# dwkim606/optimal_conv

Hardware: AMD Instinct MI355X
Metric: homomorphic convs/sec (conv_then_pack + BN bias, k x k, batch B, N=2^16) (higher is better)
Workload: dtype u64; 1 GPU; conv 3 3; ker_wid=3, batch=256, in_wid=16, logN=16, moduli=ckks.DefaultBootstrapParams[6] Q0,Q1 + P=0x1fffffffffe00001, ciphertexts_per_launch_set=4, contexts_per_gpu=4, chunk_nodes=512

## Files before the change

### optimal_conv_amd/csrc/hc_kernels.h

```cpp
#pragma once
#include "hc_arith.h"

#define HC_TPB 256
#ifndef HC_MIN_WAVES
#define HC_MIN_WAVES 4
#endif
#define HC_ROWS_LDS 4096
#define HC_COLS_LDS 4096

struct __attribute__((aligned(16))) HcTw { u64 w, ws; };

#define HC_SMALL_Q(q) ((q) < (1ull << 31))
template <bool B> struct HcBool { static constexpr bool value = B; };
template <int V> struct HcInt { static constexpr int value = V; };
#define HC_COUNT_DISPATCH(n, body) do { switch (n) { case 1: body(HcInt<1>{}); break; case 2: body(HcInt<2>{}); break; case 3: body(HcInt<3>{}); break; case 4: body(HcInt<4>{}); break; \
    case 5: body(HcInt<5>{}); break; case 6: body(HcInt<6>{}); break; case 7: body(HcInt<7>{}); break; case 8: body(HcInt<8>{}); break; default: break; } } while (0)
#define HC_LD(S32, rowptr, j) ((S32) ? hc_ld32(rowptr, j) : (rowptr)[j])
#define HC_ST(S32, rowptr, j, v) do { if (S32) hc_st32(rowptr, j, v); else (rowptr)[j] = (v); } while (0)
#define HC_ROW_DISPATCH(row32, body) do { if (row32) body(HcBool<true>{}); else body(HcBool<false>{}); } while (0)
__device__ __forceinline__ u64 hc_ld32(const u64 *row, size_t j) { return (u64)reinterpret_cast<const u32 *>(row)[j]; }
__device__ __forceinline__ void hc_st32(u64 *row, size_t j, u64 v) { reinterpret_cast<u32 *>(row)[j] = (u32)v; }
struct __attribute__((packed, aligned(4))) HcU64A4 { u64 v; };
__device__ __forceinline__ u64 hc_ldp(const u64 *row, size_t j, bool row32) {
    return reinterpret_cast<const HcU64A4 *>(reinterpret_cast<const char *>(row) + (j << (row32 ? 2 : 3)))->v & (row32 ? 0xFFFFFFFFull : ~0ull);
// ... 795 lines not shown
    const HcTw *__restrict__ c0 = A.ctc + ((size_t)z * 4 + 1) * 65536 + (size_t)HC_TILE * 4096 + t;
    const u64 *__restrict__ k = A.ker.p[z] + ((size_t)i * 2 + 1) * 65536 + (size_t)HC_TILE * 4096 + t;
    const HcQ Q = hc_q(A.m1.q);
    const HcTw wA = hc_twl_load(T1inv, HC_TILE, t);
    u64 e0[16], e1[16];
#pragma unroll
    for (int kk = 0; kk < 16; kk++) {
        const u64 kv = k[kk * 256];
        const HcTw w0 = c0[kk * 256], w1 = c0[2 * 65536 + kk * 256];
        e0[kk] = hc_shoup4(kv, w0.w, w0.ws, Q);
        e1[kk] = hc_shoup4(kv, w1.w, w1.ws, Q);
    }
    u64 *o = A.tmp + ((size_t)z * A.njobs + 2 * ch) * 65536 + (size_t)row * 256;
    hc_xchg(lds, [&](int kk) { return hc_rows_lds(kk, t); }, [&](int lo) { return hc_rows_lds(rloc, tid * 16 + lo); }, [] { __syncthreads(); }, e0, e1);
    HC_ROW_SYNC();
    if (F64) {
        const HcF64Mod m{(double)A.m1.q, 1.0 / (double)A.m1.q};
        double f0[16], f1[16];
#pragma unroll
        for (int kk = 0; kk < 16; kk++) { f0[kk] = hc_f64_reduce(hc_f64_from_u(e0[kk]), m.q, m.qinv); f1[kk] = hc_f64_reduce(hc_f64_from_u(e1[kk]), m.q, m.qinv); }
        hc_rows_inv2_f64(f0, f1, lds, T1inv, wA, row, rloc, tid, m);
#pragma unroll
        for (int hi = 0; hi < 16; hi++) { o[hi * 16 + tid] = hc_d2u(f0[hi]); o[65536 + hi * 16 + tid] = hc_d2u(f1[hi]); }
    } else {
        hc_rows_inv_twl(HcLazy<>{Q}, lds, T1inv, wA, row, rloc, tid, e0, e1);
#pragma unroll
        for (int hi = 0; hi < 16; hi++) { o[hi * 16 + tid] = e0[hi]; o[65536 + hi * 16 + tid] = e1[hi]; }
    }
}
template <int FM, int F64>
__global__ __launch_bounds__(HC_TPB, HC_W_A2) void hc_k_a2(HcLoopA A, HcTwTab T1inv, HcTwTab T0fwd) {
    __shared__ u32 lds[HC_COLS_LDS];
    __shared__ __attribute__((aligned(16))) HcTw twl[HC_COLS_TWL];
    const int t = threadIdx.x, c = t & 15, tid = t >> 4;
    u64 *base = A.tmp + (size_t)HC_JOB * 65536 + HC_TILE * 16 + c;
    const HcQ Q0 = hc_q(A.m0.q);
    const HcTw wI = hc_twc_load(T1inv, t), wF = hc_twc_load(T0fwd, t);
    u64 e[16];
#pragma unroll
    for (int lo = 0; lo < 16; lo++) e[lo] = base[(size_t)(tid * 16 + lo) * 256];
    const HcTwC tI = hc_twc_put(twl, 0, wI, t), tF = hc_twc_put(twl, 1, wF, t);
    HC_ROW_SYNC();
    if (F64) {
        const double q1 = (double)A.m1.q, hh = (double)A.h;
        const HcF64Mod m{q1, 1.0 / q1};
        double f[16];
#pragma unroll
        for (int lo = 0; lo < 16; lo++) f[lo] = hc_u2d(e[lo]);
        hc_cols_inv_f64(f, lds, T1inv, tI, c, tid, m);
#pragma unroll
        for (int hi = 0; hi < 16; hi++) {
            double v = f[hi];
            v = v > hh ? v - q1 : (v < -hh ? v + q1 : v);
            e[hi] = hc_f64_to_u_plus(v, A.m0.q);
        }
    } else {
        const HcQ Q1 = hc_q(A.m1.q);
        hc_cols_inv_twl(HcLazy<>{Q1}, lds, T1inv, tI, c, tid, e, T1inv.ninv, T1inv.w_last_ninv);
#pragma unroll
        for (int hi = 0; hi < 16; hi++) {
            const u64 v = hc_csub(hc_canon4(e[hi], Q1) + A.h, A.m1.q);
            e[hi] = hc_reduce64(v + A.negh0, A.m0.mu, Q0);
        }
    }
    __syncthreads();
    hc_cols_fwd_twl(HcLazy<FM>{Q0}, lds, T0fwd, tF, c, tid, e);
#pragma unroll
    for (int lo = 0; lo < 16; lo++) base[(size_t)(tid * 16 + lo) * 256] = e[lo];
}
template <int FM>
__global__ __launch_bounds__(HC_TPB, HC_W_A3) void hc_k_a3p(HcLoopA A, HcTwTab T0fwd) {
    __shared__ __attribute__((aligned(16))) u64 lds[HC_ROWS_LDS];
    const int t = threadIdx.x, tid = t & 15, rloc = t >> 4, row = HC_TILE * 16 + rloc;
    const int ch = HC_JOB, i = A.i0 + ch * A.norm, z = blockIdx.z;
    const u64 *__restrict__ in = A.tmp + ((size_t)z * A.njobs + 2 * ch) * 65536 + (size_t)row * 256;
    const HcTw *__restrict__ c0 = A.ctc + (size_t)z * 4 * 65536 + (size_t)HC_TILE * 4096 + t;
    const u64 *__restrict__ k = A.ker.p[z] + ((size_t)i * 2) * 65536 + (size_t)HC_TILE * 4096 + t;
    u64 *__restrict__ o = A.cts + (size_t)z * A.cts_stride + (size_t)(A.slot0 + ch * A.slot_step) * 2 * 65536 + (size_t)HC_TILE * 4096 + t;
    const HcQ Q = hc_q(A.m0.q);
    const HcTw wA = hc_twl_load(T0fwd, HC_TILE, t);
    u64 e0[16], e1[16], kv[16];
#pragma unroll
    for (int hi = 0; hi < 16; hi++) { e0[hi] = in[hi * 16 + tid]; e1[hi] = in[65536 + hi * 16 + tid]; }
#pragma unroll
    for (int kk = 0; kk < 16; kk++) kv[kk] = k[kk * 256];
    hc_rows_fwd_twl(HcLazy<FM>{Q}, lds, T0fwd, wA, row, rloc, tid, e0, e1);
    HC_ROW_SYNC();
    hc_xchg(lds, [&](int lo) { return hc_rows_lds(rloc, tid * 16 + lo); }, [&](int kk) { return hc_rows_lds(kk, t); }, [] { __syncthreads(); }, e0, e1);
#pragma unroll
    for (int b = 0; b < 16; b += HC_A3_ROWS) {
        HcTw w0[HC_A3_ROWS], w1[HC_A3_ROWS];
#pragma unroll
        for (int j = 0; j < HC_A3_ROWS; j++) { w0[j] = c0[(b + j) * 256]; w1[j] = c0[2 * 65536 + (b + j) * 256]; }
#pragma unroll
        for (int j = 0; j < HC_A3_ROWS; j++) {
            const int kk = b + j;
            const u64 a0 = hc_shoup4(kv[kk], w0[j].w, w0[j].ws, Q), a1 = hc_shoup4(kv[kk], w1[j].w, w1[j].ws, Q);
            const u64 d0 = FM == HC_FM_FREE ? a0 + HC_FREE_OFF * Q.q - e0[kk] : a0 + Q.q - hc_canon8(e0[kk], Q);
            const u64 d1 = FM == HC_FM_FREE ? a1 + HC_FREE_OFF * Q.q - e1[kk] : a1 + Q.q - hc_canon8(e1[kk], Q);
            o[kk * 256] = hc_canon4(hc_shoup4(d0, A.q1inv.w, A.q1inv.ws, Q), Q);
            o[65536 + kk * 256] = hc_canon4(hc_shoup4(d1, A.q1inv.w, A.q1inv.ws, Q), Q);
        }
    }
}

struct HcLoopB {
    const u64 *src;
    u64 *dst;
    u64 *tmpC;
    u64 *tmpE;
    u64 *tmpT;
    const HcTw *idx;
    const HcTw *evkQ;
    const HcTw *evkP;
    const u64 *idxM;
    const u64 *evkQM;
    int n0, step, norm;
    int nodes;
    size_t src_stride, dst_stride;
    HcMod m0, mp;
    HcTw pmodq;
    HcTw pinv;
    u64 mu0;
    u64 vthresh;
    u32 gal;
};
__global__ __launch_bounds__(HC_TPB, HC_W_B1) void hc_k_b1(HcLoopB B, HcTwTab T0inv) {
    __shared__ __attribute__((aligned(16))) u64 lds[HC_ROWS_LDS];
    const int t = threadIdx.x, tid = t & 15, rloc = t >> 4, row = HC_TILE * 16 + rloc;
    const int job = HC_JOB, z = job / B.nodes, node = job - z * B.nodes, i = (B.n0 + node) * B.norm;
    const size_t tile = (size_t)HC_TILE * 4096 + t;
    const u64 *__restrict__ y1 = B.src + (size_t)z * B.src_stride + ((size_t)i * 2 + 1) * 65536 + tile;
    const u64 *__restrict__ x1 = B.src + (size_t)z * B.src_stride + ((size_t)(i + B.step) * 2 + 1) * 65536 + tile;
    const HcTw *__restrict__ idx = B.idx + tile;
    const HcQ Q = hc_q(B.m0.q);
    u64 e[16], yy[16];
#pragma unroll
    for (int kk = 0; kk < 16; kk++) { e[kk] = x1[kk * 256]; yy[kk] = y1[kk * 256]; }
#pragma unroll
    for (int kk = 0; kk < 16; kk++) {
        const HcTw I = idx[kk * 256];
        e[kk] = hc_fold(yy[kk] + Q.q4 - hc_shoup4(e[kk], I.w, I.ws, Q), Q.nq4);
    }
    if (B.tmpT != nullptr) {
        u64 *__restrict__ tt = B.tmpT + (size_t)job * 65536 + tile;
#pragma unroll
        for (int kk = 0; kk < 16; kk++) tt[kk * 256] = e[kk];
    }
    hc_rows_lin_to_lo(lds, t, rloc, tid, e);
    const HcTw wA = hc_twl_load(T0inv, HC_TILE, t);
    HC_ROW_SYNC();
    hc_rows_inv(HcLazy<>{Q}, lds, T0inv, row, rloc, tid, e, &wA);
    u64 *__restrict__ o = B.tmpC + (size_t)job * 65536 + (size_t)row * 256;
#pragma unroll
    for (int hi = 0; hi < 16; hi++) o[hi * 16 + tid] = e[hi];
}
template <int FMP>
__global__ __launch_bounds__(HC_TPB, HC_W_B2) void hc_k_b2(HcLoopB B, HcTwTab T0inv, HcTwTab TPfwd) {
    __shared__ u32 lds[HC_COLS_LDS];
    __shared__ __attribute__((aligned(16))) HcTw twl[HC_COLS_TWL];
    const int t = threadIdx.x, c = t & 15, tid = t >> 4;
    u64 *base = B.tmpC + (size_t)HC_JOB * 65536 + HC_TILE * 16 + c;
    const HcQ Q0 = hc_q(B.m0.q), QP = hc_q(B.mp.q);
    const HcTw wI = hc_twc_load(T0inv, t), wF = hc_twc_load(TPfwd, t);
    u64 e[16];
#pragma unroll
    for (int lo = 0; lo < 16; lo++) e[lo] = base[(size_t)(tid * 16 + lo) * 256];
    const HcTwC tI = hc_twc_put(twl, 0, wI, t), tF = hc_twc_put(twl, 1, wF, t);
    HC_ROW_SYNC();
    hc_cols_inv_twl(HcLazy<>{Q0}, lds, T0inv, tI, c, tid, e, T0inv.ninv, T0inv.w_last_ninv);
#pragma unroll
    for (int hi = 0; hi < 16; hi++) e[hi] = hc_canon4(e[hi], Q0);
    __syncthreads();
    hc_cols_fwd_twl(HcLazy<FMP>{QP}, lds, TPfwd, tF, c, tid, e);
#pragma unroll
    for (int lo = 0; lo < 16; lo++) base[(size_t)(tid * 16 + lo) * 256] = e[lo];
}
template <int FMP>
__global__ __launch_bounds__(HC_TPB, HC_W_B3) void hc_k_b3p(HcLoopB B, HcTwTab TPfwd, HcTwTab TPinv) {
    __shared__ __attribute__((aligned(16))) u64 lds[HC_ROWS_LDS];
    const int t = threadIdx.x, tid = t & 15, rloc = t >> 4, row = HC_TILE * 16 + rloc;
    const int node = HC_JOB;
    const u64 *in = B.tmpC + (size_t)node * 65536 + (size_t)row * 256;
    const HcQ Q = hc_q(B.mp.q);
    u64 e0[16], e1[16];
    HcTw wI;
    {
        const HcTw wA = hc_twl_load(TPfwd, HC_TILE, t);
        u64 cp[16];
#pragma unroll
        for (int hi = 0; hi < 16; hi++) cp[hi] = in[hi * 16 + tid];
        hc_rows_fwd_twl(HcLazy<FMP>{Q}, lds, TPfwd, wA, row, rloc, tid, cp);
        wI = hc_twl_load(TPinv, HC_TILE, t);
        const HcTw *__restrict__ ev = B.evkP + (size_t)HC_TILE * 4096 + t;
#pragma unroll
        for (int lo = 0; lo < 16; lo++) {
            const HcTw w0 = ev[lo * 256], w1 = ev[65536 + lo * 256];
            e0[lo] = hc_shoup4(cp[lo], w0.w, w0.ws, Q);
            e1[lo] = hc_shoup4(cp[lo], w1.w, w1.ws, Q);
        }
    }
    HC_ROW_SYNC();
    hc_rows_inv_twl(HcLazy<>{Q}, lds, TPinv, wI, row, rloc, tid, e0, e1);
    u64 *o = B.tmpE + (size_t)node * 2 * 65536 + (size_t)row * 256;
#pragma unroll
    for (int hi = 0; hi < 16; hi++) { o[hi * 16 + tid] = e0[hi]; o[65536 + hi * 16 + tid] = e1[hi]; }
}
template <int FM>
__global__ __launch_bounds__(HC_TPB, HC_W_B4) void hc_k_b4(HcLoopB B, HcTwTab TPinv, HcTwTab T0fwd) {
    __shared__ u32 lds[HC_COLS_LDS];
    __shared__ __attribute__((aligned(16))) HcTw twl[HC_COLS_TWL];
    const int t = threadIdx.x, c = t & 15, tid = t >> 4;
    u64 *base = B.tmpE + (size_t)HC_JOB * 65536 + HC_TILE * 16 + c;
    const HcQ QP = hc_q(B.mp.q), Q = hc_q(B.m0.q);
    const HcTw wI = hc_twc_load(TPinv, t), wF = hc_twc_load(T0fwd, t);
    u64 e[16];
#pragma unroll
    for (int lo = 0; lo < 16; lo++) e[lo] = base[(size_t)(tid * 16 + lo) * 256];
    const HcTwC tI = hc_twc_put(twl, 0, wI, t), tF = hc_twc_put(twl, 1, wF, t);
    HC_ROW_SYNC();
    hc_cols_inv_twl<false>(HcLazy<>{QP}, lds, TPinv, tI, c, tid, e, TPinv.ninv, TPinv.w_last_ninv);
#pragma unroll
    for (int hi = 0; hi < 16; hi++) {
        const u64 yv = hc_canon4(e[hi], QP);
        u64 r = hc_shoup4(yv, B.pinv.w, B.pinv.ws, Q);
        if (yv >= B.vthresh) r += Q.q - 1;
        e[hi] = r;
    }
    __syncthreads();
    hc_cols_fwd_twl(HcLazy<FM>{Q}, lds, T0fwd, tF, c, tid, e);
#pragma unroll
    for (int lo = 0; lo < 16; lo++) base[(size_t)(tid * 16 + lo) * 256] = e[lo];
}
template <int FM, int K0>
__device__ __forceinline__ void hc_b5_terms(u64 Y, u64 T, HcTw K, u64 X, HcTw I, const HcQ &Q, u64 &t1, u64 &f) {
    const u64 q = Q.q;
    u64 g = hc_shoup4(T, K.w, K.ws, Q);
    if (FM != HC_FM_FREE) g = hc_canon4(g, Q);
    if (K0) {
        u64 m = hc_shoup4(X, I.w, I.ws, Q);
        if (FM == HC_FM_FREE) { t1 = Y + m; f = Y + Q.q4 - m + g; }
        else { m = hc_canon4(m, Q); t1 = hc_addmod(Y, m, q); f = hc_addmod(hc_submod(Y, m, q), g, q); }
    } else {
        if (FM == HC_FM_FREE) t1 = Y + Y + Q.q4 - T;
        else t1 = hc_addmod(Y, hc_submod(Y, hc_canon4(T, Q), q), q);
        f = g;
    }
}
template <int FM>
__global__ __launch_bounds__(HC_TPB, 3) void hc_k_b5(HcLoopB B, HcTwTab T0fwd, HcPtrs biases, HcPtrs outs) {
    __shared__ u64 lds[HC_ROWS_LDS];
    const int t = threadIdx.x, tid = t & 15, rloc = t >> 4, row = HC_TILE * 16 + rloc;
    const int job = HC_JOB, zn = job >> 1, k = job & 1, z = zn / B.nodes, node = zn - z * B.nodes, i = (B.n0 + node) * B.norm;
    const HcQ Q = hc_q(B.m0.q);
    const u64 q = Q.q;
    const size_t tile = (size_t)HC_TILE * 4096 + t;
    const u64 *__restrict__ in = B.tmpE + (size_t)job * 65536 + (size_t)row * 256;
    const u64 *__restrict__ yk = B.src + (size_t)z * B.src_stride + ((size_t)i * 2 + k) * 65536 + tile;
    const u64 *__restrict__ xk = B.src + (size_t)z * B.src_stride + ((size_t)(i + B.step) * 2 + k) * 65536 + tile;
    const u64 *__restrict__ tc1 = B.tmpT + (size_t)zn * 65536 + tile;
    const HcTw *__restrict__ idx = B.idx + tile;
    const HcTw *__restrict__ evk = B.evkQ + (size_t)k * 65536 + tile;
    u64 *__restrict__ o = (outs.p[z] != nullptr ? const_cast<u64 *>(outs.p[z]) + (size_t)k * 65536 : B.dst + (size_t)z * B.dst_stride + ((size_t)i * 2 + k) * 65536) + tile;
    const u64 *__restrict__ bias = (k == 0 && biases.p[z] != nullptr) ? biases.p[z] + tile : nullptr;
    u64 e[16];
#pragma unroll
    for (int hi = 0; hi < 16; hi++) e[hi] = in[hi * 16 + tid];
    hc_rows_fwd(HcLazy<FM>{Q}, lds, T0fwd, row, rloc, tid, e);
    HC_ROW_SYNC();
    hc_rows_lo_to_lin(lds, t, rloc, tid, e);
    __syncthreads();
    {
        u64 t1[16];
#pragma unroll
        for (int b = 0; b < 16; b += 4) {
            u64 Y[4], T[4], X[4]; HcTw K[4], I[4];
#pragma unroll
            for (int j = 0; j < 4; j++) {
                const int off = (b + j) * 256;
                Y[j] = yk[off]; K[j] = evk[off]; T[j] = tc1[off];
                if (k == 0) { X[j] = xk[off]; I[j] = idx[off]; } else { X[j] = 0; I[j] = K[j]; }
            }
#pragma unroll
            for (int j = 0; j < 4; j++) {
                const int kk = b + j;
                u64 f;
                if (k == 0) hc_b5_terms<FM, 1>(Y[j], T[j], K[j], X[j], I[j], Q, t1[kk], f);
                else hc_b5_terms<FM, 0>(Y[j], T[j], K[j], X[j], I[j], Q, t1[kk], f);
                if (bias != nullptr) t1[kk] = FM == HC_FM_FREE ? t1[kk] + bias[kk * 256] : hc_addmod(t1[kk], bias[kk * 256], q);
                lds[hc_rows_lds(kk, t)] = FM == HC_FM_FREE ? f + HC_FREE_OFF * q - e[kk] : hc_submod(f, hc_canon8(e[kk], Q), q);
            }
        }
        __syncthreads();
#pragma unroll
        for (int kk = 0; kk < 16; kk++) {
            const u32 srcidx = hc_perm_src((u32)((HC_TILE * 16 + kk) * 256 + t), B.gal);
            const u64 d = lds[hc_rows_lds((int)((srcidx >> 8) & 15), (int)(srcidx & 255))];
            o[kk * 256] = FM == HC_FM_FREE ? hc_reduce64(t1[kk] + d, B.m0.mu, Q) : hc_addmod(t1[kk], d, q);
        }
    }
}

#ifndef HC_B5_ROWS
#define HC_B5_ROWS 4
#endif
#ifndef HC_B5M_WAVES
#define HC_B5M_WAVES 2
#endif
template <int FM>
__device__ __forceinline__ void hc_rows_fwd2_lin(u64 (&e0)[16], u64 (&e1)[16], u64 *l0, u64 *l1, const HcTwTab &T, const HcTw &wA, int row, int rloc, int tid, int t, const HcQ &Q) {
    hc_ct_round(HcLazy<FM>{Q}, hc_twl_put(l0, wA, rloc, tid), e0, e1);
    HC_ROW_SYNC();
#pragma unroll
    for (int hi = 0; hi < 16; hi++) { const int a = hc_rows_lds(rloc, hi * 16 + tid); l0[a] = e0[hi]; l1[a] = e1[hi]; }
    HC_ROW_SYNC();
#pragma unroll
    for (int lo = 0; lo < 16; lo++) { const int a = hc_rows_lds(rloc, tid * 16 + lo); e0[lo] = l0[a]; e1[lo] = l1[a]; }
    hc_ct_round(HcLazy<FM>{Q}, HcTwB<false, HcTw>{T.rowsB + row * 256 + tid}, e0, e1);
    HC_ROW_SYNC();
#pragma unroll
    for (int lo = 0; lo < 16; lo++) { const int a = hc_rows_lds(rloc, tid * 16 + lo); l0[a] = e0[lo]; l1[a] = e1[lo]; }
    __syncthreads();
#pragma unroll
    for (int k = 0; k < 16; k++) { const int a = hc_rows_lds(k, t); e0[k] = l0[a]; e1[k] = l1[a]; }
}
template <int FM>
__global__ __launch_bounds__(HC_TPB, HC_B5M_WAVES) void hc_k_b5m(HcLoopB B, HcTwTab T0fwd, HcPtrs biases, HcPtrs outs) {
    __shared__ __attribute__((aligned(16))) u64 lds[2 * HC_ROWS_LDS];
    u64 *l0 = lds, *l1 = lds + HC_ROWS_LDS;
    const int t = threadIdx.x, tid = t & 15, rloc = t >> 4, row = HC_TILE * 16 + rloc;
    const int zn = HC_JOB, z = zn / B.nodes, node = zn - z * B.nodes, i = (B.n0 + node) * B.norm;
    const HcQ Q = hc_q(B.m0.q);
    const u64 q = Q.q, qinv = B.m0.qinv;
    const size_t tile = (size_t)HC_TILE * 4096 + t;
    const u64 *__restrict__ ys = B.src + (size_t)z * B.src_stride + (size_t)i * 2 * 65536 + tile;
    const u64 *__restrict__ xs = B.src + (size_t)z * B.src_stride + (size_t)(i + B.step) * 2 * 65536 + tile;
    const u64 *__restrict__ idx = B.idxM + tile;
    const u64 *__restrict__ evk = B.evkQM + tile;
    u64 *__restrict__ o = (outs.p[z] != nullptr ? const_cast<u64 *>(outs.p[z]) : B.dst + (size_t)z * B.dst_stride + (size_t)i * 2 * 65536) + tile;
    const u64 *__restrict__ bias = biases.p[z] != nullptr ? biases.p[z] + tile : nullptr;
    const HcTw wA = hc_twl_load(T0fwd, HC_TILE, t);
    u64 e0[16], e1[16];
    {
        const u64 *__restrict__ in = B.tmpE + (size_t)zn * 2 * 65536 + (size_t)row * 256;
#pragma unroll
        for (int hi = 0; hi < 16; hi++) { e0[hi] = in[hi * 16 + tid]; e1[hi] = in[65536 + hi * 16 + tid]; }
    }
    hc_rows_fwd2_lin<FM>(e0, e1, l0, l1, T0fwd, wA, row, rloc, tid, t, Q);
    __syncthreads();
#pragma unroll
    for (int b = 0; b < 16; b += HC_B5_ROWS) {
        u64 Y0[HC_B5_ROWS], X0[HC_B5_ROWS], Y1[HC_B5_ROWS], X1[HC_B5_ROWS], K0[HC_B5_ROWS], K1[HC_B5_ROWS], I[HC_B5_ROWS], bs[HC_B5_ROWS], s0[HC_B5_ROWS], s1[HC_B5_ROWS];
#pragma unroll
        for (int j = 0; j < HC_B5_ROWS; j++) {
            const int off = (b + j) * 256;
            Y1[j] = ys[65536 + off]; X1[j] = xs[65536 + off]; Y0[j] = ys[off]; X0[j] = xs[off]; I[j] = idx[off]; K0[j] = evk[off]; K1[j] = evk[65536 + off];
            bs[j] = bias != nullptr ? bias[off] : 0;
        }
#pragma unroll
        for (int j = 0; j < HC_B5_ROWS; j++) {
            const int kk = b + j, a = hc_rows_lds(kk, t);
            u64 m1 = hc_mont_lazy(X1[j], I[j], q, qinv), m0 = hc_mont_lazy(X0[j], I[j], q, qinv);
            const u64 T = hc_fold(Y1[j] + Q.q4 - m1, Q.nq4);
            u64 g1 = hc_mont_lazy(T, K1[j], q, qinv), g0 = hc_mont_lazy(T, K0[j], q, qinv);
            if (FM == HC_FM_FREE) {
                s1[j] = Y1[j] + m1; s0[j] = Y0[j] + m0 + bs[j];
                l1[a] = g1 + HC_FREE_OFF * q - e1[kk];
                l0[a] = Y0[j] + Q.q4 - m0 + g0 + HC_FREE_OFF * q - e0[kk];
            } else {
                m1 = hc_canon4(m1, Q); m0 = hc_canon4(m0, Q); g1 = hc_canon4(g1, Q); g0 = hc_canon4(g0, Q);
                s1[j] = hc_addmod(Y1[j], m1, q); s0[j] = hc_addmod(hc_addmod(Y0[j], m0, q), bs[j], q);
                l1[a] = hc_submod(g1, hc_canon8(e1[kk], Q), q);
                l0[a] = hc_submod(hc_addmod(hc_submod(Y0[j], m0, q), g0, q), hc_canon8(e0[kk], Q), q);
            }
        }
        __syncthreads();
#pragma unroll
        for (int j = 0; j < HC_B5_ROWS; j++) {
            const int kk = b + j;
            const u32 srcidx = hc_perm_src((u32)((HC_TILE * 16 + kk) * 256 + t), B.gal);
            const int a = hc_rows_lds(kk, (int)(srcidx & 255));
            const u64 d1 = l1[a], d0 = l0[a];
            o[65536 + kk * 256] = FM == HC_FM_FREE ? hc_reduce64(s1[j] + d1, B.m0.mu, Q) : hc_addmod(s1[j], d1, q);
            o[kk * 256] = FM == HC_FM_FREE ? hc_reduce64(s0[j] + d0, B.m0.mu, Q) : hc_addmod(s0[j], d0, q);
        }
    }
}

#define HC_STPB 256
#define HC_STILES 64
#define HC_S_LDS 1024
__device__ __forceinline__ int hc_s_addr(int line, int x) { return x * 4 + line; }
__device__ __forceinline__ int hc_s_pos(int u, int lo) { return (u & ((1 << lo) - 1)) | ((u >> lo) << (lo + 2)); }
template <bool ROWS, int D> __device__ __forceinline__ HcTw hc_s_tw_fwd(const HcTwTab &T, int x, int gline) {
    if (D >= 16) { constexpr int s = D == 128 ? 0 : D == 64 ? 1 : D == 32 ? 2 : 3; const int slot = (1 << s) - 1 + (x >> (8 - s)); return ROWS ? T.rowsA[gline * 16 + slot] : T.colsA[slot]; }
    constexpr int s = D == 8 ? 0 : D == 4 ? 1 : D == 2 ? 2 : 3; const int slot = (1 << s) - 1 + ((x & 15) >> (4 - s));
    return ROWS ? T.rowsB[gline * 256 + slot * 16 + (x >> 4)] : T.colsB[slot * 16 + (x >> 4)];
}
template <bool ROWS, int D> __device__ __forceinline__ HcTw hc_s_tw_inv(const HcTwTab &T, int x, int gline) {
    if (D <= 8) { constexpr int s = D == 1 ? 0 : D == 2 ? 1 : D == 4 ? 2 : 3; const int slot = (8 >> s) - 1 + ((x & 15) >> (s + 1)); return ROWS ? T.rowsB[gline * 256 + slot * 16 + (x >> 4)] : T.colsB[slot * 16 + (x >> 4)]; }
    constexpr int s = D == 16 ? 0 : D == 32 ? 1 : D == 64 ? 2 : 3; const int slot = (8 >> s) - 1 + (x >> (5 + s));
    return ROWS ? T.rowsA[gline * 16 + slot] : T.colsA[slot];
}
__device__ __forceinline__ void hc_s_bf_fwd(u64 &X, u64 &Y, HcTw w, const HcQ &Q) { const u64 x = hc_fold(X, Q.nq4), t = hc_shoup4(Y, w.w, w.ws, Q); X = x + t; Y = (x + Q.q4) - t; }
__device__ __forceinline__ void hc_s_bf_inv(u64 &X, u64 &Y, HcTw w, const HcQ &Q) { const u64 u = X + Y, d = (X + Q.q4) - Y; X = hc_fold(u, Q.nq4); Y = hc_shoup4(d, w.w, w.ws, Q); }
template <bool ROWS> __device__ __forceinline__ void hc_s_tw_load_fwd(HcTw (&w)[12], const HcTwTab &T, int gline, int u) {
    { const int x0 = hc_s_pos(u, 6); w[0] = hc_s_tw_fwd<ROWS, 128>(T, x0, gline); w[1] = hc_s_tw_fwd<ROWS, 64>(T, x0, gline); w[2] = hc_s_tw_fwd<ROWS, 64>(T, x0 + 128, gline); }
    { const int x0 = hc_s_pos(u, 4); w[3] = hc_s_tw_fwd<ROWS, 32>(T, x0, gline); w[4] = hc_s_tw_fwd<ROWS, 16>(T, x0, gline); w[5] = hc_s_tw_fwd<ROWS, 16>(T, x0 + 32, gline); }
    { const int x0 = hc_s_pos(u, 2); w[6] = hc_s_tw_fwd<ROWS, 8>(T, x0, gline); w[7] = hc_s_tw_fwd<ROWS, 4>(T, x0, gline); w[8] = hc_s_tw_fwd<ROWS, 4>(T, x0 + 8, gline); }
    { const int x0 = hc_s_pos(u, 0); w[9] = hc_s_tw_fwd<ROWS, 2>(T, x0, gline); w[10] = hc_s_tw_fwd<ROWS, 1>(T, x0, gline); w[11] = hc_s_tw_fwd<ROWS, 1>(T, x0 + 2, gline); }
}
template <bool ROWS> __device__ __forceinline__ void hc_s_tw_load_inv(HcTw (&w)[12], const HcTwTab &T, int gline, int u) {
    { const int x0 = hc_s_pos(u, 0); w[0] = hc_s_tw_inv<ROWS, 1>(T, x0, gline); w[1] = hc_s_tw_inv<ROWS, 1>(T, x0 + 2, gline); w[2] = hc_s_tw_inv<ROWS, 2>(T, x0, gline); }
    { const int x0 = hc_s_pos(u, 2); w[3] = hc_s_tw_inv<ROWS, 4>(T, x0, gline); w[4] = hc_s_tw_inv<ROWS, 4>(T, x0 + 8, gline); w[5] = hc_s_tw_inv<ROWS, 8>(T, x0, gline); }
    { const int x0 = hc_s_pos(u, 4); w[6] = hc_s_tw_inv<ROWS, 16>(T, x0, gline); w[7] = hc_s_tw_inv<ROWS, 16>(T, x0 + 32, gline); w[8] = hc_s_tw_inv<ROWS, 32>(T, x0, gline); }
    { const int x0 = hc_s_pos(u, 6); w[9] = hc_s_tw_inv<ROWS, 64>(T, x0, gline); w[10] = hc_s_tw_inv<ROWS, 64>(T, x0 + 128, gline); w[11] = hc_s_tw_inv<ROWS, 128>(T, x0, gline); }
}
template <int D> __device__ __forceinline__ void hc_s_round_fwd(u64 *lds, HcTw wa, HcTw wb, HcTw wc, int line, int u, const HcQ &Q) {
    constexpr int lo = D == 128 ? 6 : D == 32 ? 4 : D == 8 ? 2 : 0, H = D / 2;
    const int x0 = hc_s_pos(u, lo);
    u64 e0 = lds[hc_s_addr(line, x0)], e1 = lds[hc_s_addr(line, x0 + H)], e2 = lds[hc_s_addr(line, x0 + D)], e3 = lds[hc_s_addr(line, x0 + D + H)];
    hc_s_bf_fwd(e0, e2, wa, Q); hc_s_bf_fwd(e1, e3, wa, Q);
    hc_s_bf_fwd(e0, e1, wb, Q); hc_s_bf_fwd(e2, e3, wc, Q);
    lds[hc_s_addr(line, x0)] = e0; lds[hc_s_addr(line, x0 + H)] = e1; lds[hc_s_addr(line, x0 + D)] = e2; lds[hc_s_addr(line, x0 + D + H)] = e3;
}
template <int D, bool SCALE_LAST> __device__ __forceinline__ void hc_s_round_inv(u64 *lds, const HcTwTab &T, HcTw wa, HcTw wb, HcTw wc, int line, int u, const HcQ &Q) {
    constexpr int lo = D == 1 ? 0 : D == 4 ? 2 : D == 16 ? 4 : 6, G = 2 * D;
    const int x0 = hc_s_pos(u, lo);
    u64 e0 = lds[hc_s_addr(line, x0)], e1 = lds[hc_s_addr(line, x0 + D)], e2 = lds[hc_s_addr(line, x0 + G)], e3 = lds[hc_s_addr(line, x0 + G + D)];
    hc_s_bf_inv(e0, e1, wa, Q); hc_s_bf_inv(e2, e3, wb, Q);
    if (SCALE_LAST) {
        const u64 ua = e0 + e2, da = (e0 + Q.q4) - e2, ub = e1 + e3, db = (e1 + Q.q4) - e3;
        e0 = hc_shoup4(ua, T.ninv.w, T.ninv.ws, Q); e2 = hc_shoup4(da, T.w_last_ninv.w, T.w_last_ninv.ws, Q);
        e1 = hc_shoup4(ub, T.ninv.w, T.ninv.ws, Q); e3 = hc_shoup4(db, T.w_last_ninv.w, T.w_last_ninv.ws, Q);
    } else { hc_s_bf_inv(e0, e2, wc, Q); hc_s_bf_inv(e1, e3, wc, Q); }
    lds[hc_s_addr(line, x0)] = e0; lds[hc_s_addr(line, x0 + D)] = e1; lds[hc_s_addr(line, x0 + G)] = e2; lds[hc_s_addr(line, x0 + G + D)] = e3;
}
__device__ __forceinline__ void hc_s_pass_fwd(u64 *lds, const HcTw (&w)[12], int line, int u, const HcQ &Q) {
    hc_s_round_fwd<128>(lds, w[0], w[1], w[2], line, u, Q); __syncthreads();
    hc_s_round_fwd<32>(lds, w[3], w[4], w[5], line, u, Q); __syncthreads();
    hc_s_round_fwd<8>(lds, w[6], w[7], w[8], line, u, Q); __syncthreads();
    hc_s_round_fwd<2>(lds, w[9], w[10], w[11], line, u, Q); __syncthreads();
}
template <bool SCALE> __device__ __forceinline__ void hc_s_pass_inv(u64 *lds, const HcTwTab &T, const HcTw (&w)[12], int line, int u, const HcQ &Q) {
    hc_s_round_inv<1, false>(lds, T, w[0], w[1], w[2], line, u, Q); __syncthreads();
    hc_s_round_inv<4, false>(lds, T, w[3], w[4], w[5], line, u, Q); __syncthreads();
    hc_s_round_inv<16, false>(lds, T, w[6], w[7], w[8], line, u, Q); __syncthreads();
    hc_s_round_inv<64, SCALE>(lds, T, w[9], w[10], w[11], line, u, Q); __syncthreads();
}
#if defined(HC_EMU)
template <int LB> __device__ __forceinline__ void hc_xswap(u64 &r0, u64 &r1) {
    __shared__ u64 xch[HC_STPB];
    const int t = threadIdx.x; const bool hi = (t >> LB) & 1;
    xch[t] = hi ? r0 : r1;
    __syncthreads();
    const u64 got = xch[t ^ (1 << LB)];
    __syncthreads();
    if (hi) r0 = got; else r1 = got;
}
#else
template <int LB> __device__ __forceinline__ void hc_xswap32(u32 &a, u32 &b) {
    if (LB == 5) { auto r = __builtin_amdgcn_permlane32_swap(a, b, false, false); a = r[0]; b = r[1]; }
    else if (LB == 4) { auto r = __builtin_amdgcn_permlane16_swap(a, b, false, false); a = r[0]; b = r[1]; }
    else if (LB == 3) { const u32 a0 = a; a = __builtin_amdgcn_update_dpp(a, b, 0x128, 0xF, 0xC, false); b = __builtin_amdgcn_update_dpp(b, a0, 0x128, 0xF, 0x3, false); }
    else if (LB == 2) { const u32 a0 = a; a = __builtin_amdgcn_update_dpp(a, b, 0x114, 0xF, 0xA, false); b = __builtin_amdgcn_update_dpp(b, a0, 0x104, 0xF, 0x5, false); }
    else {
        const bool hi = (threadIdx.x >> LB) & 1;
        const u32 give = hi ? a : b;
        const u32 got = LB == 1 ? __builtin_amdgcn_mov_dpp(give, 0x4E, 0xF, 0xF, true) : __builtin_amdgcn_mov_dpp(give, 0xB1, 0xF, 0xF, true);
        if (hi) a = got; else b = got;
    }
}
template <int LB> __device__ __forceinline__ void hc_xswap(u64 &r0, u64 &r1) {
    u32 a0 = (u32)r0, a1 = (u32)(r0 >> 32), b0 = (u32)r1, b1 = (u32)(r1 >> 32);
    hc_xswap32<LB>(a0, b0); hc_xswap32<LB>(a1, b1);
    r0 = ((u64)a1 << 32) | a0; r1 = ((u64)b1 << 32) | b0;
}
#endif
template <int HB> __device__ __forceinline__ void hc_s_transpose(u64 (&e)[4]) { hc_xswap<HB>(e[0], e[2]); hc_xswap<HB>(e[1], e[3]); hc_xswap<HB - 1>(e[0], e[1]); hc_xswap<HB - 1>(e[2], e[3]); }
__device__ __forceinline__ void hc_s_pass_fwd_reg(u64 (&e)[4], const HcTw (&w)[12], const HcQ &Q) {
    hc_s_bf_fwd(e[0], e[2], w[0], Q); hc_s_bf_fwd(e[1], e[3], w[0], Q); hc_s_bf_fwd(e[0], e[1], w[1], Q); hc_s_bf_fwd(e[2], e[3], w[2], Q);
    hc_s_transpose<5>(e);
    hc_s_bf_fwd(e[0], e[2], w[3], Q); hc_s_bf_fwd(e[1], e[3], w[3], Q); hc_s_bf_fwd(e[0], e[1], w[4], Q); hc_s_bf_fwd(e[2], e[3], w[5], Q);
    hc_s_transpose<3>(e);
    hc_s_bf_fwd(e[0], e[2], w[6], Q); hc_s_bf_fwd(e[1], e[3], w[6], Q); hc_s_bf_fwd(e[0], e[1], w[7], Q); hc_s_bf_fwd(e[2], e[3], w[8], Q);
    hc_s_transpose<1>(e);
    hc_s_bf_fwd(e[0], e[2], w[9], Q); hc_s_bf_fwd(e[1], e[3], w[9], Q); hc_s_bf_fwd(e[0], e[1], w[10], Q); hc_s_bf_fwd(e[2], e[3], w[11], Q);
}
__device__ __forceinline__ void hc_s_pass_inv_reg(u64 (&e)[4], const HcTw (&w)[12], const HcQ &Q) {
    hc_s_bf_inv(e[0], e[1], w[0], Q); hc_s_bf_inv(e[2], e[3], w[1], Q); hc_s_bf_inv(e[0], e[2], w[2], Q); hc_s_bf_inv(e[1], e[3], w[2], Q);
    hc_s_transpose<1>(e);
    hc_s_bf_inv(e[0], e[1], w[3], Q); hc_s_bf_inv(e[2], e[3], w[4], Q); hc_s_bf_inv(e[0], e[2], w[5], Q); hc_s_bf_inv(e[1], e[3], w[5], Q);
    hc_s_transpose<3>(e);
    hc_s_bf_inv(e[0], e[1], w[6], Q); hc_s_bf_inv(e[2], e[3], w[7], Q); hc_s_bf_inv(e[0], e[2], w[8], Q); hc_s_bf_inv(e[1], e[3], w[8], Q);
    hc_s_transpose<5>(e);
    hc_s_bf_inv(e[0], e[1], w[9], Q); hc_s_bf_inv(e[2], e[3], w[10], Q); hc_s_bf_inv(e[0], e[2], w[11], Q); hc_s_bf_inv(e[1], e[3], w[11], Q);
}
#define HC_S_ROWS_MAP const int t = threadIdx.x, line = t >> 6, u = t & 63, grow = HC_TILE * 4 + line
#define HC_S_CTILE ((int)((blockIdx.x & 7) * 8 + (blockIdx.x >> 3)))
#define HC_S_COLS_MAP const int t = threadIdx.x, line = t & 3, u = t >> 2

__global__ __launch_bounds__(HC_STPB) void hc_k_sb1(HcLoopB B, HcTwTab T0inv) {
    HC_S_ROWS_MAP;
    const int job = HC_JOB, z = job / B.nodes, node = job - z * B.nodes, i = (B.n0 + node) * B.norm;
    const size_t tile = (size_t)HC_TILE * 1024;
    const u64 *__restrict__ y1 = B.src + (size_t)z * B.src_stride + ((size_t)i * 2 + 1) * 65536 + tile;
    const u64 *__restrict__ x1 = B.src + (size_t)z * B.src_stride + ((size_t)(i + B.step) * 2 + 1) * 65536 + tile;
    const HcTw *__restrict__ idx = B.idx + tile;
    const HcQ Q = hc_q(B.m0.q);
    HcTw w[12]; hc_s_tw_load_inv<true>(w, T0inv, grow, u);
    u64 *__restrict__ o = B.tmpC + (size_t)job * 65536 + tile;
    u64 e[4];
#pragma unroll
    for (int j = 0; j < 4; j++) {
        const int p = line * 256 + u * 4 + j; const HcTw I = idx[p];
        e[j] = hc_fold(y1[p] + Q.q4 - hc_shoup4(x1[p], I.w, I.ws, Q), Q.nq4);
    }
    hc_s_pass_inv_reg(e, w, Q);
#pragma unroll
    for (int j = 0; j < 4; j++) o[line * 256 + j * 64 + u] = e[j];
}
__global__ __launch_bounds__(HC_STPB) void hc_k_sb2(HcLoopB B, HcTwTab T0inv, HcTwTab TPfwd) {
    __shared__ u64 lds[HC_S_LDS];
    HC_S_COLS_MAP;
    u64 *base = B.tmpC + (size_t)HC_JOB * 65536 + HC_S_CTILE * 4;
    const HcQ Q0 = hc_q(B.m0.q), QP = hc_q(B.mp.q);
    HcTw w[12]; hc_s_tw_load_inv<false>(w, T0inv, 0, u);
#pragma unroll
    for (int k = 0; k < 4; k++) { const int r = k * 64 + u; lds[r * 4 + line] = base[(size_t)r * 256 + line]; }
    __syncthreads();
    hc_s_pass_inv<true>(lds, T0inv, w, line, u, Q0);
    hc_s_tw_load_fwd<false>(w, TPfwd, 0, u);
#pragma unroll
    for (int k = 0; k < 4; k++) { const int a = (k * 64 + u) * 4 + line; lds[a] = hc_canon4(lds[a], Q0); }
    __syncthreads();
    hc_s_pass_fwd(lds, w, line, u, QP);
#pragma unroll
    for (int k = 0; k < 4; k++) { const int r = k * 64 + u; base[(size_t)r * 256 + line] = lds[r * 4 + line]; }
}
__global__ __launch_bounds__(HC_STPB) void hc_k_sb3(HcLoopB B, HcTwTab TPfwd, HcTwTab TPinv) {
    HC_S_ROWS_MAP;
    const int node = HC_JOB, k = blockIdx.z;
    const size_t tile = (size_t)HC_TILE * 1024;
    const u64 *in = B.tmpC + (size_t)node * 65536 + tile;
    const HcQ Q = hc_q(B.mp.q);
    HcTw w[12]; hc_s_tw_load_fwd<true>(w, TPfwd, grow, u);
    const HcTw *__restrict__ ev = B.evkP + (size_t)k * 65536;
    u64 e[4];
#pragma unroll
    for (int j = 0; j < 4; j++) e[j] = in[line * 256 + j * 64 + u];
    hc_s_pass_fwd_reg(e, w, Q);
    hc_s_tw_load_inv<true>(w, TPinv, grow, u);
#pragma unroll
    for (int j = 0; j < 4; j++) {
        const int R = grow, C = u * 4 + j;
        const HcTw kw = ev[((R >> 4) * 16 + (C & 15)) * 256 + (R & 15) * 16 + (C >> 4)];
        e[j] = hc_shoup4(e[j], kw.w, kw.ws, Q);
    }
    hc_s_pass_inv_reg(e, w, Q);
    u64 *o = B.tmpE + ((size_t)node * 2 + k) * 65536 + tile;
#pragma unroll
    for (int j = 0; j < 4; j++) o[line * 256 + j * 64 + u] = e[j];
}
__global__ __launch_bounds__(HC_STPB) void hc_k_sb4(HcLoopB B, HcTwTab TPinv, HcTwTab T0fwd) {
    __shared__ u64 lds[HC_S_LDS];
    HC_S_COLS_MAP;
    u64 *base = B.tmpE + (size_t)HC_JOB * 65536 + HC_S_CTILE * 4;
    const HcQ QP = hc_q(B.mp.q), Q = hc_q(B.m0.q);
    HcTw w[12]; hc_s_tw_load_inv<false>(w, TPinv, 0, u);
#pragma unroll
    for (int k = 0; k < 4; k++) { const int r = k * 64 + u; lds[r * 4 + line] = base[(size_t)r * 256 + line]; }
    __syncthreads();
    hc_s_pass_inv<false>(lds, TPinv, w, line, u, QP);
    hc_s_tw_load_fwd<false>(w, T0fwd, 0, u);
#pragma unroll
    for (int k = 0; k < 4; k++) {
        const int a = (k * 64 + u) * 4 + line;
        const u64 yv = hc_canon4(lds[a], QP);
        u64 r = hc_shoup4(yv, B.pinv.w, B.pinv.ws, Q);
        if (yv >= B.vthresh) r += Q.q - 1;
        lds[a] = r;
    }
    __syncthreads();
    hc_s_pass_fwd(lds, w, line, u, Q);
#pragma unroll
    for (int k = 0; k < 4; k++) { const int r = k * 64 + u; base[(size_t)r * 256 + line] = lds[r * 4 + line]; }
}
__global__ __launch_bounds__(HC_STPB) void hc_k_sb5(HcLoopB B, HcTwTab T0fwd, HcPtrs biases, HcPtrs outs) {
    __shared__ u64 lds[HC_S_LDS];
    HC_S_ROWS_MAP;
    const int job = HC_JOB, zn = job >> 1, k = job & 1, z = zn / B.nodes, node = zn - z * B.nodes, i = (B.n0 + node) * B.norm;
    const HcQ Q = hc_q(B.m0.q);
    const size_t tile = (size_t)HC_TILE * 1024;
    const u64 *__restrict__ in = B.tmpE + (size_t)job * 65536 + tile;
    const u64 *__restrict__ ys = B.src + (size_t)z * B.src_stride + (size_t)i * 2 * 65536 + tile;
    const u64 *__restrict__ xs = B.src + (size_t)z * B.src_stride + (size_t)(i + B.step) * 2 * 65536 + tile;
    const HcTw *__restrict__ idx = B.idx + tile;
    const HcTw *__restrict__ evk = B.evkQ + (size_t)k * 65536 + tile;
    u64 *__restrict__ o = (outs.p[z] != nullptr ? const_cast<u64 *>(outs.p[z]) + (size_t)k * 65536 : B.dst + (size_t)z * B.dst_stride + ((size_t)i * 2 + k) * 65536) + tile;
    const u64 *__restrict__ bias = (k == 0 && biases.p[z] != nullptr) ? biases.p[z] + tile : nullptr;
    HcTw w[12]; hc_s_tw_load_fwd<true>(w, T0fwd, grow, u);
    u64 e[4];
#pragma unroll
    for (int j = 0; j < 4; j++) e[j] = hc_reduce64(in[line * 256 + j * 64 + u], B.m0.mu, Q);
    hc_s_pass_fwd_reg(e, w, Q);
    u64 t1[4];
#pragma unroll
    for (int j = 0; j < 4; j++) {
        const int p = line * 256 + u * 4 + j;
        const u64 nraw = e[j];
        const HcTw I = idx[p], K = evk[p];
        const u64 y1 = ys[65536 + p], x1 = xs[65536 + p];
        const u64 T = hc_fold(y1 + Q.q4 - hc_shoup4(x1, I.w, I.ws, Q), Q.nq4);
        const u64 g = hc_canon4(hc_shoup4(T, K.w, K.ws, Q), Q);
        const u64 n = hc_canon8(nraw, Q);
        u64 f;
        if (k == 0) {
            const u64 y0 = ys[p], m = hc_canon4(hc_shoup4(xs[p], I.w, I.ws, Q), Q);
            t1[j] = hc_addmod(y0, m, Q.q);
            if (bias != nullptr) t1[j] = hc_addmod(t1[j], bias[p], Q.q);
            f = hc_addmod(hc_submod(y0, m, Q.q), g, Q.q);
        } else {
            t1[j] = hc_addmod(y1, hc_submod(y1, hc_canon4(T, Q), Q.q), Q.q);
            f = g;
        }
        lds[p] = hc_submod(f, n, Q.q);
    }
    __syncthreads();
#pragma unroll
    for (int j = 0; j < 4; j++) {
        const int p = line * 256 + u * 4 + j;
        const u32 srcidx = hc_perm_src((u32)(HC_TILE * 1024 + p), B.gal);
        o[p] = hc_addmod(t1[j], lds[srcidx & 1023], Q.q);
    }
}



struct HcBasisExt {
    int n;
    u64 s[8];
    HcTw inv[8];
    HcTw hat[8];
    HcTw smodt;
    u64 t, mu_t;
    u64 mu_s[8];
};
#ifndef HC_EXT_GROUP
#define HC_EXT_GROUP 4
#endif
#define HC_MAX_NP 5
template <int NS>
__device__ __forceinline__ u64 hc_basis_ext_sum(const u64 (&y)[NS + 1], const HcBasisExt &B, const HcQ &Q) {
    const int n = B.n;
    u64 v = 0;
#pragma unroll
    for (int i = 0; i <= NS; i++) if (i == n) v = y[i];
    if (n == 1) return hc_barrett64(y[0], B.t, B.mu_t);
    const u64 vs = (u64)(u32)v * B.smodt.w;
    if (B.t < (1ull << 58)) {
        u64 acc = 2 * Q.q4, hi = 0;
#pragma unroll
        for (int i = 0; i < NS; i++) if (i < n) { acc += y[i] * B.hat[i].w; hi += hc_mulhi_lo2(y[i], B.hat[i].ws); }
        return hc_reduce64(acc + hi * Q.nq - vs, B.mu_t, Q);
    }
    u64 acc = 0;
#pragma unroll
    for (int i = 0; i < NS; i++) if (i < n) acc = hc_fold(acc + hc_shoup4(y[i], B.hat[i].w, B.hat[i].ws, Q), Q.nq4);
    return hc_canon8(acc + Q.q4 - hc_fold(vs, Q.nq4), Q);
}
template <int NS>
__device__ __forceinline__ u64 hc_basis_ext_sum_full(const u64 (&y)[NS + 1], const HcBasisExt &B, const HcQ &Q) {
    const u64 vs = (u64)(u32)y[NS] * B.smodt.w;
    if (B.t < (1ull << 58)) {
        u64 acc = 2 * Q.q4, hi = 0;
#pragma unroll
        for (int i = 0; i < NS; i++) { acc += y[i] * B.hat[i].w; hi += hc_mulhi_lo2(y[i], B.hat[i].ws); }
        return hc_reduce64(acc + hi * Q.nq - vs, B.mu_t, Q);
    }
    u64 acc = 0;
#pragma unroll
    for (int i = 0; i < NS; i++) acc = hc_fold(acc + hc_shoup4(y[i], B.hat[i].w, B.hat[i].ws, Q), Q.nq4);
    return hc_canon8(acc + Q.q4 - hc_fold(vs, Q.nq4), Q);
}
template <int NS>
// ... 1213 lines not shown
```

Baseline: 833.5 conv/s.

## Halve hc_k_b5m LDS footprint by sharing one tile between both polynomials

The fused rows-forward plus keyswitch epilogue kernel now uses a single 4096-entry LDS tile instead of two. The row transposes exchange the two polynomials in turn through a shared helper. In the epilogue the second polynomial is stored in the row-mirrored slot (kk^8), and the batch is cut to 2 rows so those slots stay disjoint. With half the shared memory, launch bounds request 4 waves instead of 2 to raise occupancy. The cost is extra barriers and serialized exchanges, plus smaller epilogue batches with less load batching.

```diff
diff --git a/optimal_conv_amd/csrc/hc_kernels.h b/optimal_conv_amd/csrc/hc_kernels.h
--- a/optimal_conv_amd/csrc/hc_kernels.h
+++ b/optimal_conv_amd/csrc/hc_kernels.h
@@ -1121,32 +1121,24 @@
 }
 
 #ifndef HC_B5_ROWS
-#define HC_B5_ROWS 4
+#define HC_B5_ROWS 2
 #endif
 #ifndef HC_B5M_WAVES
-#define HC_B5M_WAVES 2
+#define HC_B5M_WAVES 4
 #endif
+static_assert(HC_B5_ROWS <= 4 && 16 % HC_B5_ROWS == 0, "hc_k_b5m's epilogue shares one tile between the two polynomials: a batch of 8 rows needs a second barrier");
 template <int FM>
-__device__ __forceinline__ void hc_rows_fwd2_lin(u64 (&e0)[16], u64 (&e1)[16], u64 *l0, u64 *l1, const HcTwTab &T, const HcTw &wA, int row, int rloc, int tid, int t, const HcQ &Q) {
-    hc_ct_round(HcLazy<FM>{Q}, hc_twl_put(l0, wA, rloc, tid), e0, e1);
+__device__ __forceinline__ void hc_rows_fwd2_lin(u64 (&e0)[16], u64 (&e1)[16], u64 *lds, const HcTwTab &T, const HcTw &wA, int row, int rloc, int tid, int t, const HcQ &Q) {
+    hc_ct_round(HcLazy<FM>{Q}, hc_twl_put(lds, wA, rloc, tid), e0, e1);
     HC_ROW_SYNC();
-#pragma unroll
-    for (int hi = 0; hi < 16; hi++) { const int a = hc_rows_lds(rloc, hi * 16 + tid); l0[a] = e0[hi]; l1[a] = e1[hi]; }
-    HC_ROW_SYNC();
-#pragma unroll
-    for (int lo = 0; lo < 16; lo++) { const int a = hc_rows_lds(rloc, tid * 16 + lo); e0[lo] = l0[a]; e1[lo] = l1[a]; }
+    hc_xchg(lds, [&](int hi) { return hc_rows_lds(rloc, hi * 16 + tid); }, [&](int lo) { return hc_rows_lds(rloc, tid * 16 + lo); }, [] { HC_ROW_SYNC(); }, e0, e1);
     hc_ct_round(HcLazy<FM>{Q}, HcTwB<false, HcTw>{T.rowsB + row * 256 + tid}, e0, e1);
     HC_ROW_SYNC();
-#pragma unroll
-    for (int lo = 0; lo < 16; lo++) { const int a = hc_rows_lds(rloc, tid * 16 + lo); l0[a] = e0[lo]; l1[a] = e1[lo]; }
-    __syncthreads();
-#pragma unroll
-    for (int k = 0; k < 16; k++) { const int a = hc_rows_lds(k, t); e0[k] = l0[a]; e1[k] = l1[a]; }
+    hc_xchg(lds, [&](int lo) { return hc_rows_lds(rloc, tid * 16 + lo); }, [&](int kk) { return hc_rows_lds(kk, t); }, [] { __syncthreads(); }, e0, e1);
 }
 template <int FM>
 __global__ __launch_bounds__(HC_TPB, HC_B5M_WAVES) void hc_k_b5m(HcLoopB B, HcTwTab T0fwd, HcPtrs biases, HcPtrs outs) {
-    __shared__ __attribute__((aligned(16))) u64 lds[2 * HC_ROWS_LDS];
-    u64 *l0 = lds, *l1 = lds + HC_ROWS_LDS;
+    __shared__ __attribute__((aligned(16))) u64 lds[HC_ROWS_LDS];
     const int t = threadIdx.x, tid = t & 15, rloc = t >> 4, row = HC_TILE * 16 + rloc;
     const int zn = HC_JOB, z = zn / B.nodes, node = zn - z * B.nodes, i = (B.n0 + node) * B.norm;
     const HcQ Q = hc_q(B.m0.q);
@@ -1165,7 +1157,7 @@
 #pragma unroll
         for (int hi = 0; hi < 16; hi++) { e0[hi] = in[hi * 16 + tid]; e1[hi] = in[65536 + hi * 16 + tid]; }
     }
-    hc_rows_fwd2_lin<FM>(e0, e1, l0, l1, T0fwd, wA, row, rloc, tid, t, Q);
+    hc_rows_fwd2_lin<FM>(e0, e1, lds, T0fwd, wA, row, rloc, tid, t, Q);
     __syncthreads();
 #pragma unroll
     for (int b = 0; b < 16; b += HC_B5_ROWS) {
@@ -1178,19 +1170,19 @@
         }
 #pragma unroll
         for (int j = 0; j < HC_B5_ROWS; j++) {
-            const int kk = b + j, a = hc_rows_lds(kk, t);
+            const int kk = b + j, a0 = hc_rows_lds(kk, t), a1 = hc_rows_lds(kk ^ 8, t);
             u64 m1 = hc_mont_lazy(X1[j], I[j], q, qinv), m0 = hc_mont_lazy(X0[j], I[j], q, qinv);
             const u64 T = hc_fold(Y1[j] + Q.q4 - m1, Q.nq4);
             u64 g1 = hc_mont_lazy(T, K1[j], q, qinv), g0 = hc_mont_lazy(T, K0[j], q, qinv);
             if (FM == HC_FM_FREE) {
                 s1[j] = Y1[j] + m1; s0[j] = Y0[j] + m0 + bs[j];
-                l1[a] = g1 + HC_FREE_OFF * q - e1[kk];
-                l0[a] = Y0[j] + Q.q4 - m0 + g0 + HC_FREE_OFF * q - e0[kk];
+                lds[a1] = g1 + HC_FREE_OFF * q - e1[kk];
+                lds[a0] = Y0[j] + Q.q4 - m0 + g0 + HC_FREE_OFF * q - e0[kk];
             } else {
                 m1 = hc_canon4(m1, Q); m0 = hc_canon4(m0, Q); g1 = hc_canon4(g1, Q); g0 = hc_canon4(g0, Q);
                 s1[j] = hc_addmod(Y1[j], m1, q); s0[j] = hc_addmod(hc_addmod(Y0[j], m0, q), bs[j], q);
-                l1[a] = hc_submod(g1, hc_canon8(e1[kk], Q), q);
-                l0[a] = hc_submod(hc_addmod(hc_submod(Y0[j], m0, q), g0, q), hc_canon8(e0[kk], Q), q);
+                lds[a1] = hc_submod(g1, hc_canon8(e1[kk], Q), q);
+                lds[a0] = hc_submod(hc_addmod(hc_submod(Y0[j], m0, q), g0, q), hc_canon8(e0[kk], Q), q);
             }
         }
         __syncthreads();
@@ -1198,8 +1190,7 @@
         for (int j = 0; j < HC_B5_ROWS; j++) {
             const int kk = b + j;
             const u32 srcidx = hc_perm_src((u32)((HC_TILE * 16 + kk) * 256 + t), B.gal);
-            const int a = hc_rows_lds(kk, (int)(srcidx & 255));
-            const u64 d1 = l1[a], d0 = l0[a];
+            const u64 d1 = lds[hc_rows_lds(kk ^ 8, (int)(srcidx & 255))], d0 = lds[hc_rows_lds(kk, (int)(srcidx & 255))];
             o[65536 + kk * 256] = FM == HC_FM_FREE ? hc_reduce64(s1[j] + d1, B.m0.mu, Q) : hc_addmod(s1[j], d1, q);
             o[kk * 256] = FM == HC_FM_FREE ? hc_reduce64(s0[j] + d0, B.m0.mu, Q) : hc_addmod(s0[j], d0, q);
         }
```

Measured after the change: 847.0 conv/s, median of 6. 1.02x the previous value.
